# alpapad/java-rsync

Hardware: AMD Instinct MI355X
Metric: GiB/s device-resident rolling+MD5 scan (Generator block sums + Sender match scan; bytes read) (higher is better)
Workload: dtype u8

## Files before the change

include/rsync_hip_debug.h:

```cpp
#ifndef RSYNC_HIP_DEBUG_H
#define RSYNC_HIP_DEBUG_H

#include <stdint.h>

#include "rsync_hip.h"

#ifdef __cplusplus
extern "C" {
#endif

int rsh_debug_set_option(const char* name, int64_t value);
int rsh_debug_get_option(const char* name, int64_t* value);
void rsh_debug_reset_options(void);

int rsh_debug_kernel_ms(rsh_ctx* ctx, int32_t which, double* ms);

int rsh_debug_generation(rsh_ctx* ctx, int32_t set, int32_t* gen);

int rsh_debug_streams_busy(rsh_ctx* ctx, int32_t* mask);

int rsh_debug_k1_clock(rsh_ctx* ctx, const void* d_data, int64_t n, int32_t block_length, int32_t reps,
                       double* clock_ghz);

int32_t rsh_debug_k1_dma_swizzle(int32_t what, int32_t chunk, int32_t index);

int rsh_debug_multi_selftest(const int64_t* bytes, int32_t njobs, int32_t nparts, int32_t fail_part, int32_t* part_out,
                             int32_t* order_out, int32_t* status_out);

int rsh_debug_tokens_selftest(const uint8_t* src, int64_t n, const rsh_event* ev, int64_t n_ev,
                              const uint8_t file_md5[16], int64_t from, uint8_t* out, int64_t len, int64_t span,
                              int64_t* n_desc);

int rsh_debug_sums_selftest(int32_t unframe, const rsh_header* h, int32_t* weak, uint8_t* strong, uint8_t* wire,
                            int64_t len, int64_t span, int64_t* n_desc);

typedef struct {
    int64_t pos;
    int32_t kind;
    int32_t value;
// ... 13 lines not shown
```

java-rsync_amd/csrc/capi.cpp:

```cpp
#include <hip/hip_runtime.h>
#include <immintrin.h>
#include <stdio.h>
#include <stdlib.h>
#include <string.h>

#include <algorithm>
#include <atomic>
#include <chrono>
#include <functional>
#include <thread>
#include <vector>

#include "device.h"
#include "host_md5.h"
#include "resolver.h"
#include "rsync_hip.h"

#include "ctx.h"
#include "options.h"
#include "rsync_hip_debug.h"

namespace {
int warm_calls(rsh_ctx* c) {
    const uint8_t seed[4] = {1, 2, 3, 4};
// ... 478 lines not shown
    return RSH_OK;
}

int rsh_debug_get_option(const char* name, int64_t* value) {
    const int i = rsh::opt_index(name);
    if (i < 0 || !value) return RSH_E_INVAL;
    *value = rsh::opt((rsh::Opt)i);
    return RSH_OK;
}

void rsh_debug_reset_options(void) {
    for (int i = 0; i < rsh::OPT_COUNT; ++i) rsh::opt_table()[i].store(rsh::opt_info()[i].def, std::memory_order_relaxed);
}

int32_t rsh_debug_k1_dma_swizzle(int32_t what, int32_t chunk, int32_t index) {
    if (what < 0 || what > 2 || chunk < 0 || chunk > 63 || index < 0 || index > 7) return -1;
    const uint32_t c = (uint32_t)chunk, i = (uint32_t)index;
    return (int32_t)(what == 0 ? rsh::k1_dma_piece(c, i) : what == 1 ? rsh::k1_dma_slot(c, i) : rsh::k1_dma_lds_byte(c, i));
}

int rsh_debug_kernel_ms(rsh_ctx* ctx, int32_t which, double* ms) {
    if (!ctx || !ms || which < 0 || which > 2) return RSH_E_INVAL;
    *ms = -1.0;
    const bool timed = which == 0 ? ctx->gen_timed : which == 1 ? ctx->spec_timed : ctx->sums_timed;
    if (!timed) return RSH_OK;
    const hipEvent_t a = which == 0 ? ctx->ev_gen_a : which == 1 ? ctx->ev_k1a : ctx->ev_sums_a;
    const hipEvent_t b = which == 0 ? ctx->ev_gen_b : which == 1 ? ctx->ev_k1b : ctx->ev_sums_b;
    RSH_HIP(hipSetDevice(ctx->device));
    RSH_HIP(hipEventSynchronize(b));
    float f = 0.f;
    RSH_HIP(hipEventElapsedTime(&f, a, b));
    *ms = f;
    return RSH_OK;
// ... 57 lines not shown
```

java-rsync_amd/csrc/device.h:

```cpp
#pragma once
#include <hip/hip_runtime.h>
#include <stdint.h>

#include <vector>

#include "hit_cache.h"
#include "rsync_hip.h"

namespace rsh {

hipError_t launch_block_sums(const uint8_t* d_data, int64_t n, uint32_t B, uint32_t nchunks, uint32_t dl,
                             uint32_t seed_word, int32_t* d_weak, uint8_t* d_strong, hipStream_t s,
                             const int* abort_flag = nullptr, int abort_gen = 0);
void k1_timing_next(hipEvent_t start, hipEvent_t stop);
bool k1_timing_taken();

#ifdef RSH_KBENCH
hipError_t launch_block_sums_variant(int variant, const uint8_t* d_data, int64_t n, uint32_t B, uint32_t nchunks,
                                     uint32_t dl, uint32_t seed_word, int32_t* d_weak, uint8_t* d_strong,
                                     hipStream_t s, const int* abort_flag = nullptr, int abort_gen = 0);
#endif

struct K1File {
    const uint8_t* data;
// ... 46 lines not shown
    uint32_t g0, ng;
    const int* abort = nullptr;
    int32_t file = 0;
    uint32_t nfull = 0;
};
uint32_t plan_block_sums_files(const K1File* files, int32_t nfiles, std::vector<K1Plan>* plans,
                               std::vector<K1Lane>* lanes, int* lane_align, bool* partial = nullptr);
hipError_t launch_expand_groups(const K1Plan* d_plans, uint32_t nplans, uint32_t ngroups, K1Group* d_groups,
                                hipStream_t s);
bool tail_gather_on();
constexpr uint32_t K1_DMA_STAGE = 8192;
constexpr uint32_t k1_dma_piece(uint32_t c, uint32_t p) { return p ^ ((c >> 1) & 7u); }
constexpr uint32_t k1_dma_slot(uint32_t c, uint32_t k) { return k ^ ((c >> 1) & 7u); }
constexpr uint32_t k1_dma_lds_byte(uint32_t c, uint32_t slot) { return 128u * c + 16u * slot; }
bool k1_dma_on();
hipError_t launch_block_sums_batch(const K1Group* d_groups, uint32_t ngroups, const K1Lane* d_lanes, uint32_t nlanes,
                                   int lane_align, uint32_t seed_word, hipStream_t s, const int* abort_flag = nullptr,
                                   int abort_gen = 0, bool partial = false);

hipError_t launch_chain_flags(const int32_t* d_wsrc, const uint8_t* d_ssrc, const int32_t* d_wbas,
                              const uint8_t* d_sbas, uint32_t count, uint32_t dl, uint8_t* d_flags,
                              hipStream_t s);
hipError_t launch_warm_k1(hipStream_t s);
hipError_t launch_warm_scan(hipStream_t s);
hipError_t launch_warm_chain(hipStream_t s);
hipError_t launch_warm_io(hipStream_t s);
constexpr uint32_t kStampGroups = 64, kStampLine = 16;
struct Stamp {
    uint32_t* counter;
    int* stamp;
// ... 258 lines not shown
```

java-rsync_amd/csrc/device.hip:

```cpp
#include <hip/hip_ext.h>
#include <hip/hip_runtime.h>

#include "device.h"
#include "device_common.h"
#include "md5_core.h"
#include "options.h"

#include <algorithm>
#include <type_traits>

namespace rsh {

__device__ __forceinline__ void weak_block(const uint32_t (&m)[16], int32_t& s1, int32_t& u, uint32_t off) {
    int32_t a = 0, b = 0;
#pragma unroll
    for (int j = 0; j < 16; ++j) {
        a = __builtin_amdgcn_sdot4((int)m[j], 0x01010101, a, false);
        const int w = (4 * j) | ((4 * j + 1) << 8) | ((4 * j + 2) << 16) | ((4 * j + 3) << 24);
        b = __builtin_amdgcn_sdot4((int)m[j], w, b, false);
    }
    s1 += a;
    u += (int32_t)(off * (uint32_t)a) + b;
}

// ... 184 lines not shown
                                                                                          seed, e.weak, e.strong);
}

typedef int v4i32 __attribute__((ext_vector_type(4)));


__device__ __forceinline__ int poll_abort(const int* flag) {
    int v;
    asm volatile("s_load_dword %0, %1, 0x0 glc\n\ts_waitcnt lgkmcnt(0)" : "=s"(v) : "s"(flag));
    return v;
}

__device__ __forceinline__ void compiler_fence() { asm volatile("" ::: "memory"); }

__device__ __forceinline__ void md5_stream_block(Md5State& st, const uint32_t (&m)[16]) { md5_compress_rot16n(st, m); }

#ifndef RSH_K1_TAIL_PF
#define RSH_K1_TAIL_PF 2
#endif
#ifdef RSH_K1_NUMVGPR
#define K1_PIPE_ATTR __attribute__((amdgpu_num_vgpr(RSH_K1_NUMVGPR)))
#else
#define K1_PIPE_ATTR __attribute__((amdgpu_waves_per_eu(3)))
#endif
template <bool MULTI = false, bool GATHER = false, bool WEAKV = false, bool DMA = false, int DIAG = 0>
__device__ __forceinline__ void block_sums_pipe_body(const uint8_t* __restrict__ data, uint32_t B, uint32_t dl,
                                                             uint32_t seed, int32_t* __restrict__ weak_out,
                                                             uint8_t* __restrict__ strong_out,
                                                             const int* abort_flag = nullptr, int abort_gen = 0,
                                                             const K1Group* __restrict__ groups = nullptr,
// ... 89 lines not shown
                accW = __builtin_amdgcn_mfma_i32_16x16x64_i8(wW[k], b4, accW, 0, 0, 0);
            }
        }
    };
    uint4 Wa[4];
    if constexpr (DMA) {
        static_assert(!GATHER && !WEAKV, "the DMA form is the main waves' form only");
        B = (uint32_t)__builtin_amdgcn_readfirstlane((int)B);
        const uint64_t ga = reinterpret_cast<uint64_t>(gdata);
        const v4i32 desc = {__builtin_amdgcn_readfirstlane((int)(uint32_t)ga),
                            __builtin_amdgcn_readfirstlane((int)((uint32_t)(ga >> 32) & 0xFFFFu)),
                            DIAG == 1 ? 0 : (int)(64u * B),
                            0x00020000};
        const uint32_t lds0 = __builtin_amdgcn_readfirstlane(
            (int)(uint32_t)reinterpret_cast<uintptr_t>((__attribute__((address_space(3))) void*)lds_all));
        const uint32_t voff = (uint32_t)(l >> 3) * B + 16u * k1_dma_piece((uint32_t)(l >> 3), (uint32_t)(l & 7));
        const uint32_t so1 = 8u * B, so2 = 16u * B, so3 = 24u * B, so4 = 32u * B, so5 = 40u * B, so6 = 48u * B,
                       so7 = 56u * B;
        auto dma = [&](int slot, uint32_t stg) __attribute__((always_inline)) {
            uint32_t keep;
            const uint32_t ve = voff + 128u * stg, vo = ve ^ 64u;
            asm volatile(
                "s_nop 4\n\t"
                "s_waitcnt lgkmcnt(0)\n\t"
                "s_mov_b32 %0, m0\n\t"
                "s_mov_b32 m0, %4\n\t"
                "s_nop 0\n\t"
                "buffer_load_dwordx4 %2, %1, 0 offen nt lds\n\t"
                "s_add_u32 m0, m0, 0x400\n\t"
                "s_nop 0\n\t"
                "buffer_load_dwordx4 %3, %1, %5 offen nt lds\n\t"
                "s_add_u32 m0, m0, 0x400\n\t"
                "s_nop 0\n\t"
                "buffer_load_dwordx4 %2, %1, %6 offen nt lds\n\t"
                "s_add_u32 m0, m0, 0x400\n\t"
                "s_nop 0\n\t"
                "buffer_load_dwordx4 %3, %1, %7 offen nt lds\n\t"
                "s_add_u32 m0, m0, 0x400\n\t"
                "s_nop 0\n\t"
                "buffer_load_dwordx4 %2, %1, %8 offen nt lds\n\t"
                "s_add_u32 m0, m0, 0x400\n\t"
                "s_nop 0\n\t"
                "buffer_load_dwordx4 %3, %1, %9 offen nt lds\n\t"
                "s_add_u32 m0, m0, 0x400\n\t"
                "s_nop 0\n\t"
                "buffer_load_dwordx4 %2, %1, %10 offen nt lds\n\t"
                "s_add_u32 m0, m0, 0x400\n\t"
                "s_nop 0\n\t"
                "buffer_load_dwordx4 %3, %1, %11 offen nt lds\n\t"
                "s_mov_b32 m0, %0"
                : "=&s"(keep)
                : "s"(desc), "v"(ve), "v"(vo), "s"(lds0 + (uint32_t)slot * K1_DMA_STAGE), "s"(so1), "s"(so2), "s"(so3),
                  "s"(so4), "s"(so5), "s"(so6), "s"(so7)
                : "memory", "scc");
        };
        const uint32_t rdx = ((uint32_t)l >> 1) & 7u;
        auto get_stage = [&](uint4 (&w0)[4], uint4 (&w1)[4], int slot) __attribute__((always_inline)) {
#pragma unroll
            for (int k = 0; k < 4; ++k) w0[k] = lds_all[slot * 512 + 8 * l + (int)((uint32_t)k ^ rdx)];
#pragma unroll
            for (int k = 0; k < 4; ++k) w1[k] = lds_all[slot * 512 + 8 * l + (int)((uint32_t)(4 + k) ^ rdx)];
        };
        uint4 Wb[2][4];
        int flag = 0;
        auto stage = [&](auto pc, uint32_t si, bool has_next, bool refill, bool poll) __attribute__((always_inline)) {
            constexpr int P = decltype(pc)::value;
            if (refill) dma(P, si + 2);
            if (poll) asm volatile("s_load_dword %0, %1, 0x0 glc" : "=s"(flag) : "s"(abort_flag));
            md5_block(Wa);
// ... 145 lines not shown

constexpr bool k1_dma_swizzle_ok() {
    for (uint32_t k = 0; k < 8; ++k)
        for (uint32_t g = 0; g < 4; ++g) {
            uint32_t spans = 0;
            for (uint32_t i = 0; i < 16; ++i) {
                const uint32_t c = 16 * g + i, slot = k1_dma_slot(c, k);
                if (slot > 7 || k1_dma_piece(c, slot) != k) return false;
                spans |= 1u << ((k1_dma_lds_byte(c, slot) >> 4) & 15u);
            }
            if (spans != 0xFFFFu) return false;
        }
    return true;
}
static_assert(k1_dma_swizzle_ok(), "K1 DMA image: bank conflict or slot / piece mismatch");
bool k1_dma_on() { return opt(OPT_K1_DMA) != 0; }

template <bool MULTI = false>
__global__ __launch_bounds__(64) K1_PIPE_ATTR void block_sums_pipe_kernel(const uint8_t* __restrict__ data, uint32_t B, uint32_t dl,
                                                             uint32_t seed, int32_t* __restrict__ weak_out,
                                                             uint8_t* __restrict__ strong_out,
                                                             const int* abort_flag = nullptr, int abort_gen = 0,
                                                             const K1Group* __restrict__ groups = nullptr,
                                                             int64_t n = 0, uint32_t nchunks = 0,
                                                             uint32_t main_waves = 0xFFFFFFFFu) {
    block_sums_pipe_body<MULTI, false, false, true>(data, B, dl, seed, weak_out, strong_out, abort_flag, abort_gen,
                                                    groups, n, nchunks, main_waves);
}
template <bool MULTI = false>
__global__ __launch_bounds__(64) K1_PIPE_ATTR void block_sums_pipe_reg_kernel(
// ... 73 lines not shown
hipError_t launch_k1_clock(const uint8_t* d_data, int64_t n, uint32_t B, uint32_t dl, uint32_t seed_word,
                           int32_t* d_weak, uint8_t* d_strong, unsigned long long* d_clk, hipStream_t s) {
    if (B == 0 || B % 128 != 0 || n <= 0 || n % (64 * (int64_t)B) != 0 || dl > 16) return hipErrorInvalidValue;
    const uint32_t nchunks = (uint32_t)(n / B), waves = nchunks / 64;
    if (k1_dma_on() && reinterpret_cast<uintptr_t>(d_data) % 16 == 0)
        hipLaunchKernelGGL(block_sums_pipe_clock_kernel<true>, dim3(waves), dim3(64), 2 * K1_DMA_STAGE, s, d_data, B, dl,
                           seed_word, d_weak, d_strong, never_word(), -1, n, nchunks, d_clk);
    else
        hipLaunchKernelGGL(block_sums_pipe_clock_kernel<false>, dim3(waves), dim3(64), 2 * 64 * 9 * sizeof(uint4), s,
                           d_data, B, dl, seed_word, d_weak, d_strong, never_word(), -1, n, nchunks, d_clk);
    return hipGetLastError();
}
#ifndef RSH_K1_SHIFT_VGPR
#define RSH_K1_SHIFT_VGPR 256
#endif
template <int W>
__device__ __forceinline__ void shift_wave(const uint8_t* __restrict__ gdata, uint32_t a, uint32_t B, uint32_t dl,
                                           uint32_t seed, int32_t* __restrict__ weak_out,
                                           uint8_t* __restrict__ strong_out, const int* abort_flag, int abort_gen) {
    constexpr int ROW = 17;
    extern __shared__ __attribute__((aligned(16))) uint4 lds_all[];
    const int l = threadIdx.x;
    const uint32_t nst = B >> 7;
    const uint32_t Q = a >> 4, r = a & 3;
    const int wr0 = (l >> 3) * ROW + (l & 7);
    const int row = l * ROW;

    v4i32 wW[4];
    v4i32 accW = {0, 0, 0, 0}, RW = {0, 0, 0, 0};
    {
        const int m = l & 15, q = l >> 4, type = m >> 2;
#pragma unroll
        for (int w = 0; w < 4; ++w)
#pragma unroll
            for (int d = 0; d < 4; ++d) {
                uint32_t word = 0;
                if (q == (m & 3) && type == 0) word = 0x01010101u;
                else if (q == (m & 3) && type == 1)
#pragma unroll
                    for (int b = 0; b < 4; ++b) word |= (uint32_t)(16 * w + 4 * d + b) << (8 * b);
                wW[w][d] = (int)word;
            }
    }
    uint4 q[2][8];
    uint4 Wa[5];
    uint4 Wb[5];
    const __amdgpu_buffer_rsrc_t rsrc =
        __builtin_amdgcn_make_buffer_rsrc(const_cast<uint8_t*>(gdata), 0, (int)(64 * B + 128), 0x00020000);
    const uint32_t lane_off = (uint32_t)(l >> 3) * B + 16u * (uint32_t)(l & 7);
    auto load = [&](uint4 (&dst)[8], uint32_t line) __attribute__((always_inline)) {
#pragma unroll
        for (int j = 0; j < 8; ++j) {
            const u32x4 t = __builtin_amdgcn_raw_buffer_load_b128(rsrc, lane_off + 128u * line, (int)(j * 8u * B), 2);
            dst[j] = make_uint4(t.x, t.y, t.z, t.w);
        }
    };
    auto put = [&](const uint4 (&src)[8], int half) __attribute__((always_inline)) {
#pragma unroll
        for (int j = 0; j < 8; ++j) lds_all[wr0 + j * 8 * ROW + 8 * half] = src[j];
    };
    auto get_words = [&](uint4 (&w)[5], int P, int h) __attribute__((always_inline)) {
#pragma unroll
        for (int k = 0; k < 5; ++k) w[k] = lds_all[row + ((8 * P + 4 * h + Q + k) & 15)];
    };
    Md5State st = md5_init();
    auto md5_block = [&](const uint4 (&w)[5]) __attribute__((always_inline)) {
        uint32_t d[20];
#pragma unroll
        for (int k = 0; k < 5; ++k) {
            d[4 * k] = w[k].x;
            d[4 * k + 1] = w[k].y;
            d[4 * k + 2] = w[k].z;
            d[4 * k + 3] = w[k].w;
        }
        uint32_t m[16];
#pragma unroll
        for (int i = 0; i < 16; ++i) m[i] = __builtin_amdgcn_alignbyte(d[W + i + 1], d[W + i], r);
        md5_stream_block(st, m);
#pragma unroll
        for (int e = 0; e < 4; ++e) RW[e] += accW[e];
#pragma unroll
        for (int k = 0; k < 4; ++k) {
            const v4i32 b4 = {(int)m[4 * k], (int)m[4 * k + 1], (int)m[4 * k + 2], (int)m[4 * k + 3]};
            accW = __builtin_amdgcn_mfma_i32_16x16x64_i8(wW[k], b4, accW, 0, 0, 0);
        }
    };
    auto step = [&](auto pc, uint32_t u, bool prev, bool next, bool refill) __attribute__((always_inline)) {
        constexpr int P = decltype(pc)::value;
        if (prev) get_words(Wb, P ^ 1, 1);
        compiler_fence();
        if (next) {
            put(q[P ^ 1], P ^ 1);
            if (refill) load(q[P ^ 1], u + 3);
        }
        if (prev) md5_block(Wa);
        compiler_fence();
        if (next) get_words(Wa, P, 0);
        if (prev) md5_block(Wb);
        compiler_fence();
    };
// ... 5 lines not shown
    compiler_fence();
    step(std::integral_constant<int, 0>{}, 0, false, true, true);
    uint32_t u = 1;
    [[maybe_unused]] int flag = 0;
    for (; u + 4 <= nst && flag != abort_gen; u += 2) {
        asm volatile("s_load_dword %0, %1, 0x0 glc" : "=s"(flag) : "s"(abort_flag));
        step(std::integral_constant<int, 1>{}, u, true, true, true);
        step(std::integral_constant<int, 0>{}, u + 1, true, true, true);
        asm volatile("s_waitcnt lgkmcnt(0)" : "+s"(flag));
    }
    if (flag == abort_gen) return;
    for (; u <= nst; u += 2) {
        step(std::integral_constant<int, 1>{}, u, true, u < nst, u + 3 <= nst);
        if (u + 1 <= nst) step(std::integral_constant<int, 0>{}, u + 1, true, u + 1 < nst, u + 4 <= nst);
    }
    {
        const uint64_t bits = ((uint64_t)B + 4) * 8;
        uint32_t m[16] = {seed, 0x80u, 0, 0, 0, 0, 0, 0, 0, 0, 0, 0, 0, 0, (uint32_t)bits, (uint32_t)(bits >> 32)};
        md5_compress(st, m);
    }
#pragma unroll
    for (int e = 0; e < 4; ++e) RW[e] += accW[e];
    const int n = l & 15, qq = l >> 4;
    int32_t tS[4], tR[4], tW[4];
#pragma unroll
    for (int e = 0; e < 4; ++e) {
        tS[e] = __shfl(accW[e], n, 64);
        tR[e] = __shfl(RW[e], n, 64);
        tW[e] = __shfl(accW[e], n + 16, 64);
    }
    const int32_t S = qq == 0 ? tS[0] : qq == 1 ? tS[1] : qq == 2 ? tS[2] : tS[3];
    const int32_t Rq = qq == 0 ? tR[0] : qq == 1 ? tR[1] : qq == 2 ? tR[2] : tR[3];
    const int32_t Wq = qq == 0 ? tW[0] : qq == 1 ? tW[1] : qq == 2 ? tW[2] : tW[3];
    const int32_t uw = (int32_t)(64u * (2u * nst * (uint32_t)S - (uint32_t)Rq)) + Wq;
    const int32_t s2 = (int32_t)(B * (uint32_t)S - (uint32_t)uw);
    weak_out[l] = (int32_t)(((uint32_t)S & 0xFFFFu) | ((uint32_t)s2 << 16));
    store_digest(strong_out + (size_t)l * dl, st, dl);
}

template <int W>
__global__ __launch_bounds__(64) __attribute__((amdgpu_num_vgpr(RSH_K1_SHIFT_VGPR))) void block_sums_shift_kernel(
    const uint8_t* __restrict__ data, int64_t n, uint32_t a, uint32_t B, uint32_t nchunks, uint32_t main_waves,
    uint32_t dl, uint32_t seed, int32_t* __restrict__ weak_out, uint8_t* __restrict__ strong_out,
    const int* abort_flag, int abort_gen, uint32_t tail_full) {
    if (blockIdx.x >= main_waves) {
        const uint32_t tw = blockIdx.x - main_waves, ngw = (tail_full + 63u) / 64u;
        if (tw < ngw) {
            const uint32_t first = main_waves * 64u + 64u * tw;
            block_sums_pipe_body<false, true>(
                data + (size_t)first * B, B, dl, seed, weak_out + first, strong_out + (size_t)first * dl, abort_flag,
                abort_gen, nullptr, 0, 0, 0xFFFFFFFFu, nullptr, min(64u, tail_full - 64u * tw));
            return;
        }
        const uint32_t c = main_waves * 64u + tail_full + (tw - ngw) * 64u + threadIdx.x;
        if (c < nchunks) lane_chunk_sums<16, 4, false>(data, n, B, c, dl, seed, weak_out, strong_out);
        return;
    }
    const uint32_t c0 = blockIdx.x * 64u;
    shift_wave<W>(data - a + (size_t)c0 * B, a, B, dl, seed, weak_out + c0, strong_out + (size_t)c0 * dl, abort_flag,
                  abort_gen);
}

__global__ __launch_bounds__(64) __attribute__((amdgpu_num_vgpr(RSH_K1_SHIFT_VGPR))) void block_sums_seg_kernel(
    const K1Seg* __restrict__ segs, uint32_t nseg, const K1Tail* __restrict__ tails, uint32_t ntail, uint32_t B,
    uint32_t dl, uint32_t seed, uint32_t ngf, const int* never) {
    if (blockIdx.x >= nseg) {
        const uint32_t tw = blockIdx.x - nseg, ngw = (ngf + 63u) / 64u;
        if (tw < ngw) {
            block_sums_pipe_body<false, true>(nullptr, B, dl, seed, nullptr, nullptr, never, -1,
                                                               nullptr, 0, 0, 0xFFFFFFFFu, tails + 64u * tw,
                                                               min(64u, ngf - 64u * tw));
            return;
        }
        const uint32_t i = ngf + (tw - ngw) * 64u + threadIdx.x;
        if (i < ntail) {
            const K1Tail t = tails[i];
            lane_chunk_sums<0, 4, false>(t.data, t.n, B, t.c, dl, seed, t.weak, t.strong);
        }
        return;
    }
    const K1Seg g = segs[blockIdx.x];
    switch ((g.a >> 2) & 3) {
        case 0: shift_wave<0>(g.lines, g.a, B, dl, seed, g.weak, g.strong, g.abort, g.abort_gen); break;
        case 1: shift_wave<1>(g.lines, g.a, B, dl, seed, g.weak, g.strong, g.abort, g.abort_gen); break;
        case 2: shift_wave<2>(g.lines, g.a, B, dl, seed, g.weak, g.strong, g.abort, g.abort_gen); break;
        default: shift_wave<3>(g.lines, g.a, B, dl, seed, g.weak, g.strong, g.abort, g.abort_gen);
    }
}

hipError_t launch_block_sums_segments(const K1Seg* d_segs, uint32_t nseg, const K1Tail* d_tails, uint32_t ntail,
                                      uint32_t nfull, uint32_t B, uint32_t dl, uint32_t seed_word, hipStream_t s) {
    if (nseg + ntail == 0) return hipSuccess;
    const bool gather_on = tail_gather_on();
    const int* never = never_word();
    uint32_t ngf = 0;
    if (gather_on && never && nfull > 0 && nfull <= ntail && (B % 128) == 0 && (B >> 7) >= 4 &&
        (nfull + 63) / 64 + (ntail - nfull + 63) / 64 == (ntail + 63) / 64)
        ngf = nfull;
    const uint32_t waves = nseg + (ngf + 63) / 64 + (ntail - ngf + 63) / 64;
    const size_t lb = ngf > 0 ? 2 * 64 * 9 * sizeof(uint4) : 64 * 17 * sizeof(uint4);
    hipLaunchKernelGGL(block_sums_seg_kernel, dim3(waves), dim3(64), lb, s, d_segs, nseg, d_tails, ntail, B, dl,
                       seed_word, ngf, never);
    return hipGetLastError();
}


constexpr uint32_t kCUs = 256;

namespace {
thread_local hipEvent_t t_k1_start = nullptr, t_k1_stop = nullptr;
thread_local bool t_k1_taken = false;
}
void k1_timing_next(hipEvent_t start, hipEvent_t stop) {
    t_k1_start = start;
    t_k1_stop = stop;
    t_k1_taken = false;
}
// ... 54 lines not shown
                hipSuccess &&
            addr - a >= reinterpret_cast<uintptr_t>(lo)) {
            const int64_t avail = (int64_t)(reinterpret_cast<uintptr_t>(lo) + size - (addr - a));
            const uint32_t nfullc = (uint32_t)std::min<int64_t>(n / B, nchunks);
            const int64_t fit = avail >= 128 ? (avail - 128) / ((int64_t)64 * B) : 0;
            const uint32_t mw = (uint32_t)std::min<int64_t>(nfullc / 64, fit);
            if (mw > 0) {
                uint32_t tail_waves = (nchunks - 64 * mw + 63) / 64;
                const uint32_t tail_full = nfullc - 64 * mw, tail_short = nchunks - nfullc;
                const uint32_t gwaves = (tail_full + 63) / 64 + (tail_short + 63) / 64;
                const bool gather = tail_full > 0 && tail_gather_on() &&
                                    (gwaves == tail_waves || mw + gwaves <= 2 * 4 * kCUs);
                const uint32_t tf = gather ? tail_full : 0u;
                if (gather) tail_waves = gwaves;
                const dim3 grid(mw + tail_waves);
                const size_t lb = gather ? 2 * 64 * 9 * sizeof(uint4) : 64 * 17 * sizeof(uint4);
                switch ((a >> 2) & 3) {
                    case 0:
                        k1_launch(block_sums_shift_kernel<0>, grid, dim3(64), (uint32_t)lb, s, d_data, n, a, B, nchunks,
                                  mw, dl, seed_word, d_weak, d_strong, abort_flag, abort_gen, tf);
                        break;
                    case 1:
                        k1_launch(block_sums_shift_kernel<1>, grid, dim3(64), (uint32_t)lb, s, d_data, n, a, B, nchunks,
                                  mw, dl, seed_word, d_weak, d_strong, abort_flag, abort_gen, tf);
                        break;
                    case 2:
                        k1_launch(block_sums_shift_kernel<2>, grid, dim3(64), (uint32_t)lb, s, d_data, n, a, B, nchunks,
                                  mw, dl, seed_word, d_weak, d_strong, abort_flag, abort_gen, tf);
                        break;
                    default:
                        k1_launch(block_sums_shift_kernel<3>, grid, dim3(64), (uint32_t)lb, s, d_data, n, a, B, nchunks,
                                  mw, dl, seed_word, d_weak, d_strong, abort_flag, abort_gen, tf);
                }
                return hipGetLastError();
            }
        }
    }
    const uint32_t waves = (uint32_t)std::min<int64_t>(n / B, nchunks) / 64;
    if (coalesced && waves > 0 && ((addr % 16) == 0 || opt(OPT_K1_UNALIGNED) != 0)) {
        const uint32_t nfullc = (uint32_t)std::min<int64_t>(n / B, nchunks);
        const size_t wave_lds = 64 * 9 * sizeof(uint4);
        const uint32_t tail_waves = (nchunks - 64 * waves + 63) / 64;
        const uint32_t tail_full = nfullc - 64 * waves, tail_short = nchunks - nfullc;
        const uint32_t gwaves = (tail_full + 63) / 64 + (tail_short + 63) / 64;
        const bool dma = dma_on && (addr % 16) == 0;
        if (tail_full > 0 && tail_gather_on() && (gwaves == tail_waves || waves + gwaves <= 2 * 4 * kCUs)) {
            k1_launch(dma ? block_sums_pipe_tailg_kernel : block_sums_pipe_tailg_reg_kernel, dim3(waves + gwaves),
                      dim3(64), (uint32_t)(2 * wave_lds), s, d_data, B, dl, seed_word, d_weak, d_strong, abort_flag,
// ... 250 lines not shown
```

java-rsync_amd/csrc/options.h:

```cpp
#pragma once
#include <stdint.h>
#include <string.h>

#include <atomic>

namespace rsh {

enum Opt : int {
    OPT_K1_GATHER,
    OPT_K1_SHIFT,
    OPT_K1_UNALIGNED,
    OPT_SCAN_TRACE,
    OPT_SCAN_SEGMENTED,
    OPT_SCAN_SAMPLES,
    OPT_BATCH_CHAIN,
    OPT_BATCH_CHAIN_PREFIX,
    OPT_HOST_CORES,
    OPT_FILE_TILE,
    OPT_FILE_TILE_ABOVE,
    OPT_PROBE_LONG,
    OPT_SEGMENT_BYTES,
    OPT_MD5_WIDTH,
    OPT_CHAIN_HELPERS,
    OPT_CHAIN_MAP_BYTES,
    OPT_TIME_GEN,
    OPT_BATCH_WARM,
    OPT_FAULT_INJECT,
    OPT_TOKENS_SPAN,
    OPT_TOKENS_PIECE,
    OPT_SUMS_PIECE,
    OPT_TOKENS_RUNS,
    OPT_K1_DMA,
    OPT_COUNT
};

struct OptInfo {
    const char* name;
    int64_t def;
};

inline constexpr OptInfo kOpts[OPT_COUNT] = {
    {"k1_gather", 1},           {"k1_shift", 1},        {"k1_unaligned", 1},
    {"scan_trace", 0},          {"scan_segmented", 1},  {"scan_samples", 256},
    {"batch_chain", 1},         {"batch_chain_prefix", -1}, {"host_cores", 0},
    {"file_tile", 4LL << 30},   {"file_tile_above", 32LL << 30}, {"probe_long", 1},
    {"segment_bytes", 16LL << 30}, {"md5_width", 0},    {"chain_helpers", -1},
    {"chain_map_bytes", 1LL << 30}, {"time_gen", 1},    {"batch_warm", 128},
    {"fault_inject", 0},        {"tokens_span", 256LL << 10}, {"tokens_piece", 8LL << 20},
    {"sums_piece", 32LL << 20}, {"tokens_runs", 64LL << 10}, {"k1_dma", 1},
};

inline const OptInfo* opt_info() { return kOpts; }

inline std::atomic<int64_t>* opt_table() {
    static std::atomic<int64_t> v[OPT_COUNT] = {};
    static std::atomic<bool> init{false};
    if (!init.load(std::memory_order_acquire)) {
        static std::atomic_flag once = ATOMIC_FLAG_INIT;
        if (!once.test_and_set()) {
            for (int i = 0; i < OPT_COUNT; ++i) v[i].store(kOpts[i].def, std::memory_order_relaxed);
            init.store(true, std::memory_order_release);
        } else {
            while (!init.load(std::memory_order_acquire)) {
            }
// ... 15 lines not shown
```

java-rsync_amd/rsync_hip.py:

```python
import ctypes
import os
import subprocess

import numpy as np

HERE = os.path.dirname(os.path.abspath(__file__))
LIB_PATH = os.environ.get("RSH_LIB") or os.path.join(HERE, "lib", "librsynchip.so")

RSH_OK, RSH_E_INVAL, RSH_E_PROTOCOL, RSH_E_OVERFLOW, RSH_E_NOSPACE, RSH_E_DEVICE, RSH_E_NOMEM, RSH_E_BUSY = \
    0, -1, -2, -3, -4, -5, -6, -7
RSH_E_NOTFOUND, RSH_E_OPEN, RSH_E_NOSOURCE = -8, -9, -10
EV_LITERAL, EV_MATCH = 1, 2


class ProtocolError(Exception):
    """RsyncProtocolException (Connection.receiveChecksumHeader, Connection.java:28-38)."""


class FileViewNotFound(FileNotFoundError):
    """RSH_E_NOTFOUND (io/FileViewNotFound: new FileView on a missing file, FileView.java:74-75)."""


class FileViewOpenFailed(OSError):
    """RSH_E_OPEN (io/FileViewOpenFailed, FileView.java:76-78)."""
# ... 120 lines not shown
                        ("count", "<i4"), ("reserved", "<i4")])

EXPORTS = ["rsh_abi_version", "rsh_strerror", "rsh_last_error", "rsh_device_count", "rsh_ctx_create", "rsh_ctx_destroy",
           "rsh_ctx_stream", "rsh_block_length_for", "rsh_digest_length_for", "rsh_header_make",
           "rsh_header_validate", "rsh_block_sums", "rsh_block_sums_device", "rsh_ctx_sync", "rsh_ctx_trim", "rsh_match_scan",
           "rsh_match_scan_device", "rsh_match_scan_tiled", "rsh_fetch_events", "rsh_file_md5", "rsh_tokens_size", "rsh_tokens_write", "rsh_generator_bytes",
           "rsh_block_sums_batch_device", "rsh_match_scan_batch_device", "rsh_receiver_combine",
           "rsh_receiver_combine_device", "rsh_receiver_combine_batch", "rsh_block_sums_file", "rsh_match_scan_file", "rsh_block_sums_pieces", "rsh_match_scan_pieces", "rsh_block_sums_batch", "rsh_match_scan_batch", "rsh_block_sums_batch_multi", "rsh_match_scan_batch_multi", "rsh_receiver_combine_batch_multi", "rsh_shard_files", "rsh_file_md5_batch", "rsh_dev_alloc", "rsh_dev_free", "rsh_memcpy_h2d", "rsh_memcpy_d2h", "rsh_fill_splitmix_device",
           "rsh_tokens_write_device", "rsh_tokens_write_kept", "rsh_tokens_write_batch_device",
           "rsh_sums_wire_size", "rsh_header_from_wire", "rsh_sums_frame_device", "rsh_sums_unframe_device",
           "rsh_block_sums_batch_wire", "rsh_match_scan_batch_wire", "rsh_block_sums_batch_wire_multi",
           "rsh_match_scan_batch_wire_multi", "rsh_tokens_frame_device", "rsh_receiver_combine_resident"]
DEBUG_EXPORTS = ["rsh_debug_set_option", "rsh_debug_get_option", "rsh_debug_reset_options", "rsh_debug_k1_clock",
                 "rsh_debug_streams_busy", "rsh_debug_kernel_ms", "rsh_debug_multi_selftest", "rsh_debug_generation",
                 "rsh_debug_tokens_selftest", "rsh_debug_sums_selftest", "rsh_debug_tokens_scan_selftest",
                 "rsh_debug_untokens_selftest", "rsh_debug_k1_dma_swizzle"]

_LIB = None


def build(force=False):
    cmd = ["make", "-s", "-C", HERE] + (["-B"] if force else [])
    subprocess.run(cmd, check=True)


def stale_sources():
    import hashlib
    stamp = os.path.splitext(LIB_PATH)[0] + ".srchash"
    if not os.path.exists(stamp):
        return []
    out = []
# ... 63 lines not shown
        "rsh_block_sums_batch_multi": ([ctypes.POINTER(P), I32, ctypes.POINTER(BlockBatchJob), I32, P], ctypes.c_int),
        "rsh_match_scan_batch_multi": ([ctypes.POINTER(P), I32, ctypes.POINTER(ScanBatchJob), I32, P,
                                        ctypes.POINTER(ScanStats)], ctypes.c_int),
        "rsh_receiver_combine_batch_multi": ([ctypes.POINTER(P), I32, ctypes.POINTER(CombineJob), I32], ctypes.c_int),
        "rsh_shard_files": ([P, I32, I32, P], ctypes.c_int),
        "rsh_file_md5_batch": ([ctypes.POINTER(Md5Job), I32, I32], ctypes.c_int),
        "rsh_dev_alloc": ([P, I64, ctypes.POINTER(P)], ctypes.c_int),
        "rsh_dev_free": ([P, P], ctypes.c_int),
        "rsh_memcpy_h2d": ([P, P, P, I64], ctypes.c_int),
        "rsh_memcpy_d2h": ([P, P, P, I64], ctypes.c_int),
        "rsh_fill_splitmix_device": ([P, P, I64, ctypes.c_uint64, I64], ctypes.c_int),
        "rsh_debug_set_option": ([ctypes.c_char_p, I64], ctypes.c_int),
        "rsh_debug_get_option": ([ctypes.c_char_p, ctypes.POINTER(I64)], ctypes.c_int),
        "rsh_debug_reset_options": ([], None),
        "rsh_debug_k1_dma_swizzle": ([I32, I32, I32], ctypes.c_int32),
        "rsh_debug_k1_clock": ([P, P, I64, I32, I32, ctypes.POINTER(ctypes.c_double)], ctypes.c_int),
        "rsh_debug_streams_busy": ([P, ctypes.POINTER(ctypes.c_int32)], ctypes.c_int),
        "rsh_debug_generation": ([P, I32, ctypes.POINTER(ctypes.c_int32)], ctypes.c_int),
        "rsh_debug_kernel_ms": ([P, I32, ctypes.POINTER(ctypes.c_double)], ctypes.c_int),
        "rsh_debug_multi_selftest": ([P, I32, I32, I32, P, P, P], ctypes.c_int),
        "rsh_tokens_write_device": ([P, P, I64, P, I64, P, I64, P, I64], ctypes.c_int),
        "rsh_tokens_write_kept": ([P, P, I64, P, I64, P, I64], ctypes.c_int),
        "rsh_tokens_write_batch_device": ([P, ctypes.POINTER(TokenJob), I32], ctypes.c_int),
        "rsh_debug_tokens_selftest": ([P, I64, P, I64, P, I64, P, I64, I64, ctypes.POINTER(I64)], ctypes.c_int),
        "rsh_sums_wire_size": ([HP], I64),
        "rsh_header_from_wire": ([P, HP], ctypes.c_int),
        "rsh_sums_frame_device": ([P, HP, P, P, P, I64], ctypes.c_int),
        "rsh_sums_unframe_device": ([P, HP, P, I64, P, P], ctypes.c_int),
        "rsh_block_sums_batch_wire": ([P, ctypes.POINTER(BlockWireJob), I32, P], ctypes.c_int),
        "rsh_match_scan_batch_wire": ([P, ctypes.POINTER(SendJob), I32, P, ctypes.POINTER(ScanStats)], ctypes.c_int),
# ... 714 lines not shown
```

Baseline: 5200.

## Feed the shifted block-sums kernel with direct-to-LDS buffer DMA ring

Adds a DMA variant of the misaligned-offset (shift) block-sums wave. It fills a double-buffered LDS image with buffer_load ... lds instructions, the same swizzled layout used by the aligned K1 path. Words are then read through a 16-slot ring that handles the byte shift, which replaces the old register-staged global loads and LDS row writes. The variant is enabled by default through a new option, and the change includes a host selftest and a static_assert that check the ring addressing. The intent is to take global-to-LDS staging off the VGPRs and overlap it with the MD5 and MFMA work. The cost is hand-written inline asm with waitcnt ordering, which is fragile.

```diff
diff --git a/include/rsync_hip_debug.h b/include/rsync_hip_debug.h
--- a/include/rsync_hip_debug.h
+++ b/include/rsync_hip_debug.h
@@ -23,6 +23,8 @@
                        double* clock_ghz);
 
 int32_t rsh_debug_k1_dma_swizzle(int32_t what, int32_t chunk, int32_t index);
+
+int32_t rsh_debug_k1_shift_dma_selftest(int32_t a, int32_t nst);
 
 int rsh_debug_multi_selftest(const int64_t* bytes, int32_t njobs, int32_t nparts, int32_t fail_part, int32_t* part_out,
                              int32_t* order_out, int32_t* status_out);
diff --git a/java-rsync_amd/csrc/capi.cpp b/java-rsync_amd/csrc/capi.cpp
--- a/java-rsync_amd/csrc/capi.cpp
+++ b/java-rsync_amd/csrc/capi.cpp
@@ -516,9 +516,72 @@
 }
 
 int32_t rsh_debug_k1_dma_swizzle(int32_t what, int32_t chunk, int32_t index) {
+    if (what == 4 && chunk >= 0 && chunk <= 63 && index >= 0 && index <= 15)
+        return (int32_t)rsh::k1_shift_lds_byte((uint32_t)chunk, (uint32_t)index);
     if (what < 0 || what > 2 || chunk < 0 || chunk > 63 || index < 0 || index > 7) return -1;
     const uint32_t c = (uint32_t)chunk, i = (uint32_t)index;
     return (int32_t)(what == 0 ? rsh::k1_dma_piece(c, i) : what == 1 ? rsh::k1_dma_slot(c, i) : rsh::k1_dma_lds_byte(c, i));
+}
+
+int32_t rsh_debug_k1_shift_dma_selftest(int32_t a_in, int32_t nst_in) {
+    if (a_in < 0 || a_in > 127 || nst_in < 4 || nst_in > 1024) return -1;
+    const uint32_t a = (uint32_t)a_in, nst = (uint32_t)nst_in, B = 128u * nst;
+    const uint32_t Q = a >> 4, W = (a >> 2) & 3u, r = a & 3u;
+    const size_t span = (size_t)64 * B + 128;
+    std::vector<uint8_t> g(span);
+    uint64_t x = 0x5EED5EED00005D00ull + a + ((uint64_t)nst << 8);
+    for (auto& b : g) {
+        x = x * 6364136223846793005ull + 1442695040888963407ull;
+        b = (uint8_t)(x >> 56);
+    }
+    std::vector<uint8_t> lds(2 * rsh::K1_DMA_STAGE, 0xEE);
+    bool in_range = true;
+    auto fill = [&](uint32_t img, uint32_t line) {
+        for (uint32_t j = 0; j < 8; ++j)
+            for (uint32_t l = 0; l < 64; ++l) {
+                const uint32_t ve = rsh::k1_dma_fill_voff(l, B) + 128u * line;
+                const size_t src = (size_t)((j & 1u) ? ve ^ 64u : ve) + (size_t)8 * j * B;
+                if (src + 16 > span) {
+                    in_range = false;
+                    continue;
+                }
+                memcpy(&lds[img * rsh::K1_DMA_STAGE + 1024u * j + 16u * l], &g[src], 16);
+            }
+    };
+    std::vector<uint32_t> D[2] = {std::vector<uint32_t>(64 * 36), std::vector<uint32_t>(64 * 36)};
+    auto get_stage = [&](uint32_t P) {
+        for (uint32_t c = 0; c < 64; ++c)
+            for (uint32_t j = 0; j < 9; ++j) {
+                const uint32_t h = j < 4 ? 0u : 1u;
+                memcpy(&D[P][c * 36 + 4 * j], &lds[rsh::k1_shift_lds_byte(c, rsh::k1_shift_ring(P, h, Q, j - 4u * h))], 16);
+            }
+    };
+    auto block_ok = [&](uint32_t P, uint32_t t, uint32_t h) {
+        for (uint32_t c = 0; c < 64; ++c) {
+            const uint32_t* d = &D[P][c * 36 + 16 * h];
+            for (uint32_t i = 0; i < 16; ++i) {
+                const uint32_t m = (uint32_t)((((uint64_t)d[W + i + 1] << 32) | d[W + i]) >> (8 * r));
+                uint32_t want;
+                memcpy(&want, &g[a + (size_t)c * B + 128u * t + 64u * h + 4u * i], 4);
+                if (m != want) return false;
+            }
+        }
+        return true;
+    };
+    fill(0, 0);
+    fill(1, 1);
+    get_stage(0);
+    fill(0, 2);
+    for (uint32_t t = 0; t < nst; ++t) {
+        const uint32_t P = t & 1u;
+        if (!block_ok(P, t, 0)) return (int32_t)(1 + 2 * t);
+        if (t + 1 < nst) {
+            get_stage(P ^ 1u);
+            if (t + 3 <= nst) fill(P ^ 1u, t + 3);
+        }
+        if (!block_ok(P, t, 1)) return (int32_t)(2 + 2 * t);
+    }
+    return in_range ? 0 : -2;
 }
 
 int rsh_debug_kernel_ms(rsh_ctx* ctx, int32_t which, double* ms) {
diff --git a/java-rsync_amd/csrc/device.h b/java-rsync_amd/csrc/device.h
--- a/java-rsync_amd/csrc/device.h
+++ b/java-rsync_amd/csrc/device.h
@@ -84,6 +84,12 @@
 constexpr uint32_t k1_dma_slot(uint32_t c, uint32_t k) { return k ^ ((c >> 1) & 7u); }
 constexpr uint32_t k1_dma_lds_byte(uint32_t c, uint32_t slot) { return 128u * c + 16u * slot; }
 bool k1_dma_on();
+constexpr uint32_t k1_dma_fill_voff(uint32_t l, uint32_t B) { return (l >> 3) * B + 16u * k1_dma_piece(l >> 3, l & 7u); }
+constexpr uint32_t k1_shift_ring(uint32_t P, uint32_t h, uint32_t Q, uint32_t k) { return (8u * P + 4u * h + Q + k) & 15u; }
+constexpr uint32_t k1_shift_lane(uint32_t c) { return 128u * c | 16u * ((c >> 1) & 7u); }
+constexpr uint32_t k1_shift_ring_term(uint32_t i) { return 16u * (i & 7u) | K1_DMA_STAGE * (i >> 3); }
+constexpr uint32_t k1_shift_lds_byte(uint32_t c, uint32_t i) { return k1_shift_lane(c) ^ k1_shift_ring_term(i); }
+bool k1_shift_dma_on();
 hipError_t launch_block_sums_batch(const K1Group* d_groups, uint32_t ngroups, const K1Lane* d_lanes, uint32_t nlanes,
                                    int lane_align, uint32_t seed_word, hipStream_t s, const int* abort_flag = nullptr,
                                    int abort_gen = 0, bool partial = false);
diff --git a/java-rsync_amd/csrc/device.hip b/java-rsync_amd/csrc/device.hip
--- a/java-rsync_amd/csrc/device.hip
+++ b/java-rsync_amd/csrc/device.hip
@@ -222,6 +222,44 @@
 __device__ __forceinline__ void compiler_fence() { asm volatile("" ::: "memory"); }
 
 __device__ __forceinline__ void md5_stream_block(Md5State& st, const uint32_t (&m)[16]) { md5_compress_rot16n(st, m); }
+
+__device__ __forceinline__ void k1_dma_fill(const v4i32& desc, uint32_t ve, uint32_t m0v, const uint32_t (&so)[7]) {
+    uint32_t keep;
+    const uint32_t vo = ve ^ 64u;
+    asm volatile(
+        "s_nop 4\n\t"
+        "s_waitcnt lgkmcnt(0)\n\t"
+        "s_mov_b32 %0, m0\n\t"
+        "s_mov_b32 m0, %4\n\t"
+        "s_nop 0\n\t"
+        "buffer_load_dwordx4 %2, %1, 0 offen nt lds\n\t"
+        "s_add_u32 m0, m0, 0x400\n\t"
+        "s_nop 0\n\t"
+        "buffer_load_dwordx4 %3, %1, %5 offen nt lds\n\t"
+        "s_add_u32 m0, m0, 0x400\n\t"
+        "s_nop 0\n\t"
+        "buffer_load_dwordx4 %2, %1, %6 offen nt lds\n\t"
+        "s_add_u32 m0, m0, 0x400\n\t"
+        "s_nop 0\n\t"
+        "buffer_load_dwordx4 %3, %1, %7 offen nt lds\n\t"
+        "s_add_u32 m0, m0, 0x400\n\t"
+        "s_nop 0\n\t"
+        "buffer_load_dwordx4 %2, %1, %8 offen nt lds\n\t"
+        "s_add_u32 m0, m0, 0x400\n\t"
+        "s_nop 0\n\t"
+        "buffer_load_dwordx4 %3, %1, %9 offen nt lds\n\t"
+        "s_add_u32 m0, m0, 0x400\n\t"
+        "s_nop 0\n\t"
+        "buffer_load_dwordx4 %2, %1, %10 offen nt lds\n\t"
+        "s_add_u32 m0, m0, 0x400\n\t"
+        "s_nop 0\n\t"
+        "buffer_load_dwordx4 %3, %1, %11 offen nt lds\n\t"
+        "s_mov_b32 m0, %0"
+        : "=&s"(keep)
+        : "s"(desc), "v"(ve), "v"(vo), "s"(m0v), "s"(so[0]), "s"(so[1]), "s"(so[2]), "s"(so[3]), "s"(so[4]), "s"(so[5]),
+          "s"(so[6])
+        : "memory", "scc");
+}
 
 #ifndef RSH_K1_TAIL_PF
 #define RSH_K1_TAIL_PF 2
@@ -341,45 +379,10 @@
                             0x00020000};
         const uint32_t lds0 = __builtin_amdgcn_readfirstlane(
             (int)(uint32_t)reinterpret_cast<uintptr_t>((__attribute__((address_space(3))) void*)lds_all));
-        const uint32_t voff = (uint32_t)(l >> 3) * B + 16u * k1_dma_piece((uint32_t)(l >> 3), (uint32_t)(l & 7));
-        const uint32_t so1 = 8u * B, so2 = 16u * B, so3 = 24u * B, so4 = 32u * B, so5 = 40u * B, so6 = 48u * B,
-                       so7 = 56u * B;
+        const uint32_t voff = k1_dma_fill_voff((uint32_t)l, B);
+        const uint32_t so[7] = {8u * B, 16u * B, 24u * B, 32u * B, 40u * B, 48u * B, 56u * B};
         auto dma = [&](int slot, uint32_t stg) __attribute__((always_inline)) {
-            uint32_t keep;
-            const uint32_t ve = voff + 128u * stg, vo = ve ^ 64u;
-            asm volatile(
-                "s_nop 4\n\t"
-                "s_waitcnt lgkmcnt(0)\n\t"
-                "s_mov_b32 %0, m0\n\t"
-                "s_mov_b32 m0, %4\n\t"
-                "s_nop 0\n\t"
-                "buffer_load_dwordx4 %2, %1, 0 offen nt lds\n\t"
-                "s_add_u32 m0, m0, 0x400\n\t"
-                "s_nop 0\n\t"
-                "buffer_load_dwordx4 %3, %1, %5 offen nt lds\n\t"
-                "s_add_u32 m0, m0, 0x400\n\t"
-                "s_nop 0\n\t"
-                "buffer_load_dwordx4 %2, %1, %6 offen nt lds\n\t"
-                "s_add_u32 m0, m0, 0x400\n\t"
-                "s_nop 0\n\t"
-                "buffer_load_dwordx4 %3, %1, %7 offen nt lds\n\t"
-                "s_add_u32 m0, m0, 0x400\n\t"
-                "s_nop 0\n\t"
-                "buffer_load_dwordx4 %2, %1, %8 offen nt lds\n\t"
-                "s_add_u32 m0, m0, 0x400\n\t"
-                "s_nop 0\n\t"
-                "buffer_load_dwordx4 %3, %1, %9 offen nt lds\n\t"
-                "s_add_u32 m0, m0, 0x400\n\t"
-                "s_nop 0\n\t"
-                "buffer_load_dwordx4 %2, %1, %10 offen nt lds\n\t"
-                "s_add_u32 m0, m0, 0x400\n\t"
-                "s_nop 0\n\t"
-                "buffer_load_dwordx4 %3, %1, %11 offen nt lds\n\t"
-                "s_mov_b32 m0, %0"
-                : "=&s"(keep)
-                : "s"(desc), "v"(ve), "v"(vo), "s"(lds0 + (uint32_t)slot * K1_DMA_STAGE), "s"(so1), "s"(so2), "s"(so3),
-                  "s"(so4), "s"(so5), "s"(so6), "s"(so7)
-                : "memory", "scc");
+            k1_dma_fill(desc, voff + 128u * stg, lds0 + (uint32_t)slot * K1_DMA_STAGE, so);
         };
         const uint32_t rdx = ((uint32_t)l >> 1) & 7u;
         auto get_stage = [&](uint4 (&w0)[4], uint4 (&w1)[4], int slot) __attribute__((always_inline)) {
@@ -555,6 +558,14 @@
     return true;
 }
 static_assert(k1_dma_swizzle_ok(), "K1 DMA image: bank conflict or slot / piece mismatch");
+constexpr bool k1_shift_ring_ok() {
+    for (uint32_t i = 0; i < 16; ++i)
+        for (uint32_t c = 0; c < 64; ++c)
+            if (k1_shift_lds_byte(c, i) != K1_DMA_STAGE * (i >> 3) + k1_dma_lds_byte(c, k1_dma_slot(c, i & 7u)))
+                return false;
+    return true;
+}
+static_assert(k1_shift_ring_ok(), "shift kernel's DMA images: a ring slot off the pipelined K1's slot of its piece");
 bool k1_dma_on() { return opt(OPT_K1_DMA) != 0; }
 
 template <bool MULTI = false>
@@ -658,7 +669,7 @@
 #ifndef RSH_K1_SHIFT_VGPR
 #define RSH_K1_SHIFT_VGPR 256
 #endif
-template <int W>
+template <int W, bool DMA = false>
 __device__ __forceinline__ void shift_wave(const uint8_t* __restrict__ gdata, uint32_t a, uint32_t B, uint32_t dl,
                                            uint32_t seed, int32_t* __restrict__ weak_out,
                                            uint8_t* __restrict__ strong_out, const int* abort_flag, int abort_gen) {
@@ -667,8 +678,6 @@
     const int l = threadIdx.x;
     const uint32_t nst = B >> 7;
     const uint32_t Q = a >> 4, r = a & 3;
-    const int wr0 = (l >> 3) * ROW + (l & 7);
-    const int row = l * ROW;
 
     v4i32 wW[4];
     v4i32 accW = {0, 0, 0, 0}, RW = {0, 0, 0, 0};
@@ -686,6 +695,98 @@
                 wW[w][d] = (int)word;
             }
     }
+    Md5State st = md5_init();
+    auto md5_block = [&](const uint4* w) __attribute__((always_inline)) {
+        uint32_t d[20];
+#pragma unroll
+        for (int k = 0; k < 5; ++k) {
+            d[4 * k] = w[k].x;
+            d[4 * k + 1] = w[k].y;
+            d[4 * k + 2] = w[k].z;
+            d[4 * k + 3] = w[k].w;
+        }
+        uint32_t m[16];
+#pragma unroll
+        for (int i = 0; i < 16; ++i) m[i] = __builtin_amdgcn_alignbyte(d[W + i + 1], d[W + i], r);
+        md5_stream_block(st, m);
+#pragma unroll
+        for (int e = 0; e < 4; ++e) RW[e] += accW[e];
+#pragma unroll
+        for (int k = 0; k < 4; ++k) {
+            const v4i32 b4 = {(int)m[4 * k], (int)m[4 * k + 1], (int)m[4 * k + 2], (int)m[4 * k + 3]};
+            accW = __builtin_amdgcn_mfma_i32_16x16x64_i8(wW[k], b4, accW, 0, 0, 0);
+        }
+    };
+    if constexpr (DMA) {
+        B = (uint32_t)__builtin_amdgcn_readfirstlane((int)B);
+        const uint32_t Qs = (uint32_t)__builtin_amdgcn_readfirstlane((int)Q);
+        const uint64_t ga = reinterpret_cast<uint64_t>(gdata);
+        const v4i32 desc = {__builtin_amdgcn_readfirstlane((int)(uint32_t)ga),
+                            __builtin_amdgcn_readfirstlane((int)((uint32_t)(ga >> 32) & 0xFFFFu)),
+                            (int)(64u * B + 128u),
+                            0x00020000};
+        const uint32_t lds0 = __builtin_amdgcn_readfirstlane(
+            (int)(uint32_t)reinterpret_cast<uintptr_t>((__attribute__((address_space(3))) void*)lds_all));
+        const uint32_t voff = k1_dma_fill_voff((uint32_t)l, B);
+        const uint32_t so[7] = {8u * B, 16u * B, 24u * B, 32u * B, 40u * B, 48u * B, 56u * B};
+        auto fill = [&](int img, uint32_t line) __attribute__((always_inline)) {
+            k1_dma_fill(desc, voff + 128u * line, lds0 + (uint32_t)img * K1_DMA_STAGE, so);
+        };
+        uint32_t rt[2][9];
+#pragma unroll
+        for (int P = 0; P < 2; ++P)
+#pragma unroll
+            for (int j = 0; j < 9; ++j) {
+                const uint32_t h = j < 4 ? 0u : 1u;
+                rt[P][j] = k1_shift_ring_term(k1_shift_ring((uint32_t)P, h, Qs, (uint32_t)j - 4u * h));
+            }
+        const uint32_t lc = k1_shift_lane((uint32_t)l);
+        const uint8_t* lds_bytes = reinterpret_cast<const uint8_t*>(lds_all);
+        auto get_stage = [&](uint4 (&d)[9], int P) __attribute__((always_inline)) {
+#pragma unroll
+            for (int j = 0; j < 9; ++j) d[j] = *reinterpret_cast<const uint4*>(lds_bytes + (lc ^ rt[P][j]));
+        };
+        uint4 D[2][9];
+        int flag = 0;
+        auto stage = [&](auto pc, uint32_t t, bool next, bool refill, bool poll) __attribute__((always_inline)) {
+            constexpr int P = decltype(pc)::value;
+            md5_block(&D[P][0]);
+            compiler_fence();
+            if (next) {
+                asm volatile("s_waitcnt vmcnt(0)" : "+v"(st.a) : : "memory");
+                get_stage(D[P ^ 1], P ^ 1);
+                __builtin_amdgcn_sched_barrier(0);
+                if (refill) fill(P ^ 1, t + 3);
+                if (poll) asm volatile("s_load_dword %0, %1, 0x0 glc" : "=s"(flag) : "s"(abort_flag));
+                __builtin_amdgcn_sched_barrier(0);
+            }
+            md5_block(&D[P][4]);
+            compiler_fence();
+        };
+        fill(0, 0);
+        fill(1, 1);
+        asm volatile("s_waitcnt vmcnt(0)" ::: "memory");
+        get_stage(D[0], 0);
+        __builtin_amdgcn_sched_barrier(0);
+        fill(0, 2);
+        uint32_t t = 0;
+        for (; t + 4 <= nst && flag != abort_gen; t += 2) {
+            stage(std::integral_constant<int, 0>{}, t, true, true, true);
+            stage(std::integral_constant<int, 1>{}, t + 1, true, true, false);
+            asm volatile("s_waitcnt lgkmcnt(0)" : "+s"(flag));
+        }
+        if (flag == abort_gen) {
+            asm volatile("s_waitcnt vmcnt(0)" ::: "memory");
+            return;
+        }
+        for (; t < nst; t += 2) {
+            stage(std::integral_constant<int, 0>{}, t, t + 1 < nst, t + 3 <= nst, false);
+            if (t + 1 < nst) stage(std::integral_constant<int, 1>{}, t + 1, t + 2 < nst, t + 4 <= nst, false);
+        }
+        asm volatile("s_waitcnt vmcnt(0)" ::: "memory");
+    } else {
+    const int wr0 = (l >> 3) * ROW + (l & 7);
+    const int row = l * ROW;
     uint4 q[2][8];
     uint4 Wa[5];
     uint4 Wb[5];
@@ -706,28 +807,6 @@
     auto get_words = [&](uint4 (&w)[5], int P, int h) __attribute__((always_inline)) {
 #pragma unroll
         for (int k = 0; k < 5; ++k) w[k] = lds_all[row + ((8 * P + 4 * h + Q + k) & 15)];
-    };
-    Md5State st = md5_init();
-    auto md5_block = [&](const uint4 (&w)[5]) __attribute__((always_inline)) {
-        uint32_t d[20];
-#pragma unroll
-        for (int k = 0; k < 5; ++k) {
-            d[4 * k] = w[k].x;
-            d[4 * k + 1] = w[k].y;
-            d[4 * k + 2] = w[k].z;
-            d[4 * k + 3] = w[k].w;
-        }
-        uint32_t m[16];
-#pragma unroll
-        for (int i = 0; i < 16; ++i) m[i] = __builtin_amdgcn_alignbyte(d[W + i + 1], d[W + i], r);
-        md5_stream_block(st, m);
-#pragma unroll
-        for (int e = 0; e < 4; ++e) RW[e] += accW[e];
-#pragma unroll
-        for (int k = 0; k < 4; ++k) {
-            const v4i32 b4 = {(int)m[4 * k], (int)m[4 * k + 1], (int)m[4 * k + 2], (int)m[4 * k + 3]};
-            accW = __builtin_amdgcn_mfma_i32_16x16x64_i8(wW[k], b4, accW, 0, 0, 0);
-        }
     };
     auto step = [&](auto pc, uint32_t u, bool prev, bool next, bool refill) __attribute__((always_inline)) {
         constexpr int P = decltype(pc)::value;
@@ -763,6 +842,7 @@
         step(std::integral_constant<int, 1>{}, u, true, u < nst, u + 3 <= nst);
         if (u + 1 <= nst) step(std::integral_constant<int, 0>{}, u + 1, true, u + 1 < nst, u + 4 <= nst);
     }
+    }
     {
         const uint64_t bits = ((uint64_t)B + 4) * 8;
         uint32_t m[16] = {seed, 0x80u, 0, 0, 0, 0, 0, 0, 0, 0, 0, 0, 0, 0, (uint32_t)bits, (uint32_t)(bits >> 32)};
@@ -787,7 +867,7 @@
     store_digest(strong_out + (size_t)l * dl, st, dl);
 }
 
-template <int W>
+template <int W, bool DMA>
 __global__ __launch_bounds__(64) __attribute__((amdgpu_num_vgpr(RSH_K1_SHIFT_VGPR))) void block_sums_shift_kernel(
     const uint8_t* __restrict__ data, int64_t n, uint32_t a, uint32_t B, uint32_t nchunks, uint32_t main_waves,
     uint32_t dl, uint32_t seed, int32_t* __restrict__ weak_out, uint8_t* __restrict__ strong_out,
@@ -806,10 +886,11 @@
         return;
     }
     const uint32_t c0 = blockIdx.x * 64u;
-    shift_wave<W>(data - a + (size_t)c0 * B, a, B, dl, seed, weak_out + c0, strong_out + (size_t)c0 * dl, abort_flag,
-                  abort_gen);
-}
-
+    shift_wave<W, DMA>(data - a + (size_t)c0 * B, a, B, dl, seed, weak_out + c0, strong_out + (size_t)c0 * dl,
+                       abort_flag, abort_gen);
+}
+
+template <bool DMA>
 __global__ __launch_bounds__(64) __attribute__((amdgpu_num_vgpr(RSH_K1_SHIFT_VGPR))) void block_sums_seg_kernel(
     const K1Seg* __restrict__ segs, uint32_t nseg, const K1Tail* __restrict__ tails, uint32_t ntail, uint32_t B,
     uint32_t dl, uint32_t seed, uint32_t ngf, const int* never) {
@@ -830,11 +911,17 @@
     }
     const K1Seg g = segs[blockIdx.x];
     switch ((g.a >> 2) & 3) {
-        case 0: shift_wave<0>(g.lines, g.a, B, dl, seed, g.weak, g.strong, g.abort, g.abort_gen); break;
-        case 1: shift_wave<1>(g.lines, g.a, B, dl, seed, g.weak, g.strong, g.abort, g.abort_gen); break;
-        case 2: shift_wave<2>(g.lines, g.a, B, dl, seed, g.weak, g.strong, g.abort, g.abort_gen); break;
-        default: shift_wave<3>(g.lines, g.a, B, dl, seed, g.weak, g.strong, g.abort, g.abort_gen);
-    }
+        case 0: shift_wave<0, DMA>(g.lines, g.a, B, dl, seed, g.weak, g.strong, g.abort, g.abort_gen); break;
+        case 1: shift_wave<1, DMA>(g.lines, g.a, B, dl, seed, g.weak, g.strong, g.abort, g.abort_gen); break;
+        case 2: shift_wave<2, DMA>(g.lines, g.a, B, dl, seed, g.weak, g.strong, g.abort, g.abort_gen); break;
+        default: shift_wave<3, DMA>(g.lines, g.a, B, dl, seed, g.weak, g.strong, g.abort, g.abort_gen);
+    }
+}
+
+bool k1_shift_dma_on() { return opt(OPT_K1_SHIFT_DMA) != 0; }
+static size_t shift_lds_bytes(bool dma, bool gathered) {
+    const size_t body = dma ? 2 * K1_DMA_STAGE : 64 * 17 * sizeof(uint4);
+    return gathered ? std::max<size_t>(body, 2 * 64 * 9 * sizeof(uint4)) : body;
 }
 
 hipError_t launch_block_sums_segments(const K1Seg* d_segs, uint32_t nseg, const K1Tail* d_tails, uint32_t ntail,
@@ -847,9 +934,10 @@
         (nfull + 63) / 64 + (ntail - nfull + 63) / 64 == (ntail + 63) / 64)
         ngf = nfull;
     const uint32_t waves = nseg + (ngf + 63) / 64 + (ntail - ngf + 63) / 64;
-    const size_t lb = ngf > 0 ? 2 * 64 * 9 * sizeof(uint4) : 64 * 17 * sizeof(uint4);
-    hipLaunchKernelGGL(block_sums_seg_kernel, dim3(waves), dim3(64), lb, s, d_segs, nseg, d_tails, ntail, B, dl,
-                       seed_word, ngf, never);
+    const bool dma = k1_shift_dma_on();
+    const size_t lb = shift_lds_bytes(dma, ngf > 0);
+    hipLaunchKernelGGL(dma ? block_sums_seg_kernel<true> : block_sums_seg_kernel<false>, dim3(waves), dim3(64), lb, s,
+                       d_segs, nseg, d_tails, ntail, B, dl, seed_word, ngf, never);
     return hipGetLastError();
 }
 
@@ -934,24 +1022,19 @@
                 const uint32_t tf = gather ? tail_full : 0u;
                 if (gather) tail_waves = gwaves;
                 const dim3 grid(mw + tail_waves);
-                const size_t lb = gather ? 2 * 64 * 9 * sizeof(uint4) : 64 * 17 * sizeof(uint4);
-                switch ((a >> 2) & 3) {
-                    case 0:
-                        k1_launch(block_sums_shift_kernel<0>, grid, dim3(64), (uint32_t)lb, s, d_data, n, a, B, nchunks,
-                                  mw, dl, seed_word, d_weak, d_strong, abort_flag, abort_gen, tf);
-                        break;
-                    case 1:
-                        k1_launch(block_sums_shift_kernel<1>, grid, dim3(64), (uint32_t)lb, s, d_data, n, a, B, nchunks,
-                                  mw, dl, seed_word, d_weak, d_strong, abort_flag, abort_gen, tf);
-                        break;
-                    case 2:
-                        k1_launch(block_sums_shift_kernel<2>, grid, dim3(64), (uint32_t)lb, s, d_data, n, a, B, nchunks,
-                                  mw, dl, seed_word, d_weak, d_strong, abort_flag, abort_gen, tf);
-                        break;
-                    default:
-                        k1_launch(block_sums_shift_kernel<3>, grid, dim3(64), (uint32_t)lb, s, d_data, n, a, B, nchunks,
-                                  mw, dl, seed_word, d_weak, d_strong, abort_flag, abort_gen, tf);
-                }
+                const bool sdma = k1_shift_dma_on();
+                const size_t lb = shift_lds_bytes(sdma, gather);
+                auto* const kernel =
+                    sdma ? (((a >> 2) & 3) == 0   ? block_sums_shift_kernel<0, true>
+                            : ((a >> 2) & 3) == 1 ? block_sums_shift_kernel<1, true>
+                            : ((a >> 2) & 3) == 2 ? block_sums_shift_kernel<2, true>
+                                                  : block_sums_shift_kernel<3, true>)
+                         : (((a >> 2) & 3) == 0   ? block_sums_shift_kernel<0, false>
+                            : ((a >> 2) & 3) == 1 ? block_sums_shift_kernel<1, false>
+                            : ((a >> 2) & 3) == 2 ? block_sums_shift_kernel<2, false>
+                                                  : block_sums_shift_kernel<3, false>);
+                k1_launch(kernel, grid, dim3(64), (uint32_t)lb, s, d_data, n, a, B, nchunks, mw, dl, seed_word, d_weak,
+                          d_strong, abort_flag, abort_gen, tf);
                 return hipGetLastError();
             }
         }
diff --git a/java-rsync_amd/csrc/options.h b/java-rsync_amd/csrc/options.h
--- a/java-rsync_amd/csrc/options.h
+++ b/java-rsync_amd/csrc/options.h
@@ -31,6 +31,7 @@
     OPT_SUMS_PIECE,
     OPT_TOKENS_RUNS,
     OPT_K1_DMA,
+    OPT_K1_SHIFT_DMA,
     OPT_COUNT
 };
 
@@ -48,6 +49,7 @@
     {"chain_map_bytes", 1LL << 30}, {"time_gen", 1},    {"batch_warm", 128},
     {"fault_inject", 0},        {"tokens_span", 256LL << 10}, {"tokens_piece", 8LL << 20},
     {"sums_piece", 32LL << 20}, {"tokens_runs", 64LL << 10}, {"k1_dma", 1},
+    {"k1_shift_dma", 1},
 };
 
 inline const OptInfo* opt_info() { return kOpts; }
diff --git a/java-rsync_amd/rsync_hip.py b/java-rsync_amd/rsync_hip.py
--- a/java-rsync_amd/rsync_hip.py
+++ b/java-rsync_amd/rsync_hip.py
@@ -158,7 +158,8 @@
 DEBUG_EXPORTS = ["rsh_debug_set_option", "rsh_debug_get_option", "rsh_debug_reset_options", "rsh_debug_k1_clock",
                  "rsh_debug_streams_busy", "rsh_debug_kernel_ms", "rsh_debug_multi_selftest", "rsh_debug_generation",
                  "rsh_debug_tokens_selftest", "rsh_debug_sums_selftest", "rsh_debug_tokens_scan_selftest",
-                 "rsh_debug_untokens_selftest", "rsh_debug_k1_dma_swizzle"]
+                 "rsh_debug_untokens_selftest", "rsh_debug_k1_dma_swizzle",
+                 "rsh_debug_k1_shift_dma_selftest"]
 
 _LIB = None
 
@@ -252,6 +253,7 @@
         "rsh_debug_get_option": ([ctypes.c_char_p, ctypes.POINTER(I64)], ctypes.c_int),
         "rsh_debug_reset_options": ([], None),
         "rsh_debug_k1_dma_swizzle": ([I32, I32, I32], ctypes.c_int32),
+        "rsh_debug_k1_shift_dma_selftest": ([I32, I32], ctypes.c_int32),
         "rsh_debug_k1_clock": ([P, P, I64, I32, I32, ctypes.POINTER(ctypes.c_double)], ctypes.c_int),
         "rsh_debug_streams_busy": ([P, ctypes.POINTER(ctypes.c_int32)], ctypes.c_int),
         "rsh_debug_generation": ([P, I32, ctypes.POINTER(ctypes.c_int32)], ctypes.c_int),
```

After: 5200 (median of 2 runs). No clear change (+0.0%).
